# cbrl/BNN-PYNQ

Measured on AMD Instinct MI355X. Metric: images/sec (whole node) CNV-W1A1 CIFAR-10-shape batch, higher is better.
Workload: dtype u1; 1 GPU; cnvW1A1, 131072 synthetic 32x32x3 uint8 images per GPU per step, inputs resident in HBM, params cifar10/cnvW1A1; parallelism=dp1 (batch shards, no data-path collective)

## Files before the change

bnn-pynq_amd/csrc/kernels.hip:

```cpp
#include <hip/hip_runtime.h>
#include <hip/hip_ext.h>
#include <stdint.h>

#include <cstdlib>
#include <cstring>
#include <type_traits>

#define BNN_HD __host__ __device__
#include "act_faults.h"
#include "input_faults.h"
#include "kernels.h"
#include "mem_faults.h"
#include "mem_org.h"
#include "packed_params.h"
static_assert(bnn::kL0TileOffset == (int)bnn::kL0MfmaTileOffset && bnn::kL0BigBytes == (int)bnn::kL0MfmaBigBytes,
              "k_conv0_tile's operand offsets must be the ones packed_params.cpp writes the layer-0 table by");

namespace bnn {
namespace {

typedef const uint32_t __attribute__((address_space(4))) *kptr32;
typedef const uint64_t __attribute__((address_space(4))) *kptr64;

constexpr int kBlock = 256;
// ... 465 lines not shown
      for (int kx = 0; kx < 3; kx++) {
        v8i b[4];
#pragma unroll
        for (int y = 0; y < 4; y++) {
          const uint4 v = P[(2 * r + y) * 30 + cc + kx];
          b[y] = v8i{(int)v.x, (int)v.y, (int)v.z, (int)v.w, 0, 0, 0, 0};
        }
#pragma unroll
        for (int ky = 0; ky < 3; ky++)
#pragma unroll
          for (int mt = 0; mt < 2; mt++)
#pragma unroll
            for (int pt = 0; pt < 2; pt++)
              acc[mt][pt] = __builtin_amdgcn_mfma_scale_f32_32x32x64_f8f6f4(wreg[ky * 3 + kx][mt], b[ky + pt], acc[mt][pt], 4, 4, 0,
                                                                              0x7F7F7F7F, 0, 0x7F7F7F7F);
      }
      uint32_t word[2];
#pragma unroll
      for (int mt = 0; mt < 2; mt++) {
        int v[16];
#pragma unroll
        for (int k = 0; k < 16; k++) v[k] = __float_as_int(fmaxf(acc[mt][0][k], acc[mt][1][k]));
        const uint32_t nf = or_halves(sign_nibbles(v, h));
        const uint32_t pooled = nf & (uint32_t)__builtin_amdgcn_mov_dpp((int)nf, 0xB1, 0xF, 0xF, true);
        word[mt] = ~pooled;
      }
      if (h == 0 && c < 28 && !(c & 1))
        *reinterpret_cast<uint2 *>(out + ((size_t)(img0 + i) * 196 + r * 14 + (c >> 1)) * 2) = make_uint2(word[0], word[1]);
    }
  }
}

constexpr int conv_mfma_row_stride(int win) {
  int ws = win;
  while ((2 * ws - (win - 2)) % 16) ws++;
  return ws;
}
constexpr int conv_mfma_img_stride(int win, int cd) {
  const int ws = conv_mfma_row_stride(win);
  int s = cd * win * ws;
  while ((s - 2 * ((win - 2) / 2 - 1) * ws - (win - 2)) % 16) s++;
  return s;
}

template <int WIN, int CD, int NT, bool POOL, int G>
__global__ __launch_bounds__(256, 2) void k_conv_mfma(const uint32_t *__restrict__ in, uint32_t *__restrict__ out,
                                                       const uint8_t *__restrict__ tab, int n_images) {
  constexpr int WOUT = WIN - 2, RP = WOUT / 2, IPI = RP * WOUT, KH = CD / 2, KS = 9 * KH, NS = 3 * KH, STREAMS = 4 / NT;
  constexpr int PIX = WIN * WIN, DWI = PIX * CD, NPF = (G * DWI + 255) / 256;
  constexpr int WS = conv_mfma_row_stride(WIN), PIXS = WIN * WS, IMGS = conv_mfma_img_stride(WIN, CD);
  static_assert(WOUT % 2 == 0 && IPI % 2 == 0 && (NT == 2 || NT == 4), "tile geometry");
  __shared__ uint4 plane[G * IMGS];
  __shared__ uint32_t lut[256];
  const int tid = threadIdx.x, lane = tid & 63, wave = __builtin_amdgcn_readfirstlane(tid >> 6), mt = wave % NT, c = lane & 31, h = lane >> 5;
  lut[tid] = fp4_pm1((uint32_t)tid);
  const uint4 *__restrict__ wt = reinterpret_cast<const uint4 *>(tab);
  v8i wreg[KS];
#pragma unroll
  for (int ks = 0; ks < KS; ks++) {
    const uint4 v = wt[(ks * NT + mt) * 64 + lane];
    wreg[ks] = v8i{(int)v.x, (int)v.y, (int)v.z, (int)v.w, 0, 0, 0, 0};
  }
  const v16f seed = reinterpret_cast<const v16f *>(tab + (size_t)KS * NT * 64 * 16)[mt * 2 + h];
  const int ngroups = (n_images + G - 1) / G;
  uint32_t pre[NPF];
  auto fetch = [&](int grp) {
    const int img0 = grp * G, lim = min(G, n_images - img0) * DWI;
#pragma unroll
    for (int j = 0; j < NPF; j++) {
      const int d = tid + 256 * j;
      pre[j] = d < lim ? in[(size_t)img0 * DWI + d] : 0u;
    }
  };
  auto slot = [&](int d) {
    const int i = d / DWI, e = d - i * DWI, pix = e / CD, q = e % CD;
    return i * IMGS + q * PIXS + (WS == WIN ? pix : pix / WIN * WS + pix % WIN);
  };
  constexpr int STEP = 32 * STREAMS, DR = STEP / WOUT, DX = STEP % WOUT, PS_LAST = (G - 1) * IMGS + 2 * (RP - 1) * WS + WOUT - 1;
  constexpr bool RAGGED = (G * IPI) % 32 != 0;
  static_assert(DX % 2 == 0 && DR + 1 <= RP, "a lane's column keeps its parity; one row-pair wrap and one image wrap per step");
  const int item0 = (wave / NT) * 32 + c, i0 = item0 / IPI, rem0 = item0 - i0 * IPI, rp0 = rem0 / WOUT, x0 = rem0 - rp0 * WOUT;
  const int ps0 = i0 * IMGS + 2 * rp0 * WS + x0;
  const uint32_t ob0 = (uint32_t)((i0 * (WOUT * WOUT) + (2 * rp0 + h) * WOUT + x0) * NT + mt) * 4;
  if (blockIdx.x < ngroups) fetch(blockIdx.x);
  for (int grp = blockIdx.x; grp < ngroups; grp += gridDim.x) {
    const int img0 = grp * G, nimg = min(G, n_images - img0), nitems = nimg * IPI;
    uint32_t *__restrict__ gout = out + (size_t)img0 * (POOL ? RP * RP : WOUT * WOUT) * NT;
    __syncthreads();
#pragma unroll
    for (int j = 0; j < NPF; j++) {
      const int d = tid + 256 * j;
      if (d < nimg * DWI) {
        const uint32_t bits = pre[j];
        plane[slot(d)] = make_uint4(lut[bits & 255], lut[(bits >> 8) & 255], lut[(bits >> 16) & 255], lut[bits >> 24]);
      }
    }
    if (grp + (int)gridDim.x < ngroups) fetch(grp + gridDim.x);
    __syncthreads();
    int x = x0, rp = rp0, ps = ps0;
    [[maybe_unused]] uint32_t ob = ob0;
    for (int t0 = (wave / NT) * 32; t0 < nitems; t0 += STEP) {
      v16f acc[2] = {seed, seed};
      const uint4 *__restrict__ P = &plane[(RAGGED ? min(ps, PS_LAST) : ps) + h * PIXS];
      auto read = [&](v8i &b, int s, int y) {
        const uint4 v = P[(s / 3) * 2 * PIXS + y * WS + s % 3];
        b = v8i{(int)v.x, (int)v.y, (int)v.z, (int)v.w, 0, 0, 0, 0};
      };
      auto mfma = [&](const v8i (&b)[4], int s, int k) {
        acc[k & 1] = __builtin_amdgcn_mfma_scale_f32_32x32x64_f8f6f4(wreg[((k >> 1) * 3 + s % 3) * KH + s / 3], b[(k >> 1) + (k & 1)], acc[k & 1], 4,
                                                                    4, 0, 0x7F7F7F7F, 0, 0x7F7F7F7F);
      };
      v8i b[2][4];
#pragma unroll
      for (int y = 0; y < 4; y++) read(b[0][y], 0, y);
#pragma unroll
      for (int s = 0; s < NS; s++)
#pragma unroll
        for (int k = 0; k < 6; k++) {
          __builtin_amdgcn_sched_barrier(0);
          mfma(b[s & 1], s, k);
          if (s + 1 < NS && k < 4) read(b[(s + 1) & 1][k], s + 1, k);
        }
      __builtin_amdgcn_sched_barrier(0);
      const bool valid = t0 + c < nitems;
      if constexpr (POOL) {
        int v[16];
#pragma unroll
        for (int k = 0; k < 16; k++) v[k] = __float_as_int(acc[0][k]) & __float_as_int(acc[1][k]);
        const uint32_t nf = or_halves(sign_nibbles(v, h));
        const uint32_t pooled = nf & (uint32_t)__builtin_amdgcn_mov_dpp((int)nf, 0xB1, 0xF, 0xF, true);
        if (valid && h == 0 && !(c & 1)) gout[(size_t)(t0 >> 1) * NT + (c >> 1) * NT + mt] = ~pooled;
      } else {
        uint32_t nf[2];
#pragma unroll
        for (int dy = 0; dy < 2; dy++) {
          int v[16];
#pragma unroll
          for (int k = 0; k < 16; k++) v[k] = __float_as_int(acc[dy][k]);
          nf[dy] = sign_nibbles(v, h);
        }
        const auto sw = __builtin_amdgcn_permlane32_swap(nf[0], nf[1], false, false);
        if (valid) *reinterpret_cast<uint32_t *>(reinterpret_cast<char *>(gout) + ob) = ~(sw[0] | sw[1]);
      }
      x += DX, rp += DR, ps += 2 * DR * WS + DX;
      if constexpr (!POOL) ob += (2 * DR * WOUT + DX) * NT * 4;
      if (x >= WOUT) {
        x -= WOUT, rp += 1, ps += 2 * WS - WOUT;
        if constexpr (!POOL) ob += WOUT * NT * 4;
      }
      if (rp >= RP) rp -= RP, ps += IMGS - 2 * RP * WS;
    }
  }
}

__global__ __launch_bounds__(256) void k_conv_mfma_table(const uint32_t *__restrict__ rows, int row_dw, int ksteps, int tiles,
                                                          int mw, uint8_t *__restrict__ dst) {
  const int idx = blockIdx.x * 256 + threadIdx.x, nw = ksteps * tiles * 64;
  if (idx < nw) {
    const int ks = idx / (tiles * 64), mt = (idx / 64) % tiles, lane = idx & 63, n = 32 * mt + (lane & 31), h = lane >> 5;
    const uint32_t bits = rows[(size_t)n * row_dw + 2 + 2 * ks + h];
    reinterpret_cast<uint4 *>(dst)[idx] = make_uint4(fp4_pm1(bits & 255), fp4_pm1((bits >> 8) & 255), fp4_pm1((bits >> 16) & 255),
                                                     fp4_pm1(bits >> 24));
  } else if (idx < nw + tiles * 32) {
    const int j = idx - nw, mt = j >> 5, h = (j >> 4) & 1, reg = j & 15;
    const int n = 32 * mt + (reg & 3) + 8 * (reg >> 2) + 4 * h;
    long long t = (int)rows[(size_t)n * row_dw];
    t = t < -1 ? -1 : (t > mw + 2 ? mw + 2 : t);
    reinterpret_cast<float *>(dst + (size_t)nw * 16)[j] = (float)(-(mw - 2 * t) - 1);
  }
}

__device__ __forceinline__ uint32_t nibble_spread(uint32_t byte) {
  uint32_t t = byte & 0xFFu;
  t = (t | (t << 12)) & 0x000F000Fu;
  t = (t | (t << 6)) & 0x03030303u;
  return (t | (t << 3)) & 0x11111111u;
}
__device__ __forceinline__ uint4 fp4_planes(const uint32_t *lutz, const uint32_t *luts, uint32_t sg, uint32_t nz) {
  const uint32_t m = sg & nz;
  return make_uint4(lutz[nz & 255] | luts[m & 255], lutz[(nz >> 8) & 255] | luts[(m >> 8) & 255],
                    lutz[(nz >> 16) & 255] | luts[(m >> 16) & 255], lutz[nz >> 24] | luts[m >> 24]);
}
__device__ __forceinline__ void not_fired(const v16f &acc, const v16f &dt, int h, uint32_t &n0, uint32_t &n1) {
  int v[16], u[16];
#pragma unroll
  for (int k = 0; k < 16; k++) {
    v[k] = __float_as_int(acc[k]);
    u[k] = __float_as_int(acc[k] - dt[k]);
  }
  n0 = or_halves(sign_nibbles(v, h));
  n1 = or_halves(sign_nibbles(u, h));
}

template <int WIN, int CD, int NT, bool POOL, int G>
__global__ __launch_bounds__(256, 2) void k_conv_mfma_a2(const uint4 *__restrict__ in, uint32_t *__restrict__ out,
                                                          const uint8_t *__restrict__ tab, int n_images) {
  constexpr int WOUT = WIN - 2, RP = WOUT / 2, IPI = RP * WOUT, KH = CD / 2, KS = 9 * KH, STREAMS = 4 / NT;
  constexpr int PIX = WIN * WIN, QWI = PIX * KH, NPF = (G * QWI + 255) / 256;
  static_assert(WOUT % 2 == 0 && IPI % 2 == 0 && (NT == 2 || NT == 4), "tile geometry");
  __shared__ uint4 plane[G][CD][PIX];
  __shared__ uint32_t lutz[256], luts[256];
  const int tid = threadIdx.x, lane = tid & 63, wave = tid >> 6, mt = wave % NT, c = lane & 31, h = lane >> 5;
  lutz[tid] = nibble_spread((uint32_t)tid) << 1;
  luts[tid] = nibble_spread((uint32_t)tid) << 3;
  const uint4 *__restrict__ wt = reinterpret_cast<const uint4 *>(tab);
  v8i wreg[KS];
#pragma unroll
  for (int ks = 0; ks < KS; ks++) {
    const uint4 v = wt[(ks * NT + mt) * 64 + lane];
    wreg[ks] = v8i{(int)v.x, (int)v.y, (int)v.z, (int)v.w, 0, 0, 0, 0};
  }
  const v16f *__restrict__ cst = reinterpret_cast<const v16f *>(tab + (size_t)KS * NT * 64 * 16);
  const v16f seed = cst[mt * 2 + h], dt = cst[NT * 2 + mt * 2 + h];
  const int ngroups = (n_images + G - 1) / G;
  uint4 pre[NPF];
  auto fetch = [&](int grp) {
    const int img0 = grp * G, lim = min(G, n_images - img0) * QWI;
#pragma unroll
    for (int j = 0; j < NPF; j++) {
      const int d = tid + 256 * j;
      pre[j] = d < lim ? in[(size_t)img0 * QWI + d] : make_uint4(0u, 0u, 0u, 0u);
    }
  };
  if (blockIdx.x < ngroups) fetch(blockIdx.x);
  for (int grp = blockIdx.x; grp < ngroups; grp += gridDim.x) {
    const int img0 = grp * G, nimg = min(G, n_images - img0), nitems = nimg * IPI;
    __syncthreads();
#pragma unroll
    for (int j = 0; j < NPF; j++) {
      const int d = tid + 256 * j;
      if (d < nimg * QWI) {
        const int i = d / QWI, e = d - i * QWI, pix = e / KH, cw = e % KH;
        const uint4 v = pre[j];
        plane[i][2 * cw][pix] = fp4_planes(lutz, luts, v.x, v.z);
        plane[i][2 * cw + 1][pix] = fp4_planes(lutz, luts, v.y, v.w);
      }
    }
    if (grp + (int)gridDim.x < ngroups) fetch(grp + gridDim.x);
    __syncthreads();
    for (int t0 = (wave / NT) * 32; t0 < nitems; t0 += 32 * STREAMS) {
      const int item = min(t0 + c, nitems - 1);
      const int i = item / IPI, rem = item - i * IPI, rp = rem / WOUT, x = rem - rp * WOUT;
      v16f acc[2] = {seed, seed};
#pragma unroll
      for (int kh = 0; kh < KH; kh++) {
        const uint4 *__restrict__ P = &plane[i][kh * 2 + h][2 * rp * WIN + x];
#pragma unroll
        for (int kx = 0; kx < 3; kx++) {
          v8i b[4];
#pragma unroll
          for (int y = 0; y < 4; y++) {
            const uint4 v = P[y * WIN + kx];
            b[y] = v8i{(int)v.x, (int)v.y, (int)v.z, (int)v.w, 0, 0, 0, 0};
          }
#pragma unroll
          for (int ky = 0; ky < 3; ky++)
#pragma unroll
            for (int dy = 0; dy < 2; dy++)
              acc[dy] = __builtin_amdgcn_mfma_scale_f32_32x32x64_f8f6f4(wreg[(ky * 3 + kx) * KH + kh], b[ky + dy], acc[dy], 4, 4, 0,
                                                                         0x7F7F7F7F, 0, 0x7F7F7F7F);
        }
      }
      const bool valid = t0 + c < nitems;
      const size_t img = (size_t)(img0 + i);
      if constexpr (POOL) {
        v16f top;
#pragma unroll
        for (int k = 0; k < 16; k++) top[k] = fmaxf(acc[0][k], acc[1][k]);
        uint32_t n0, n1;
        not_fired(top, dt, h, n0, n1);
        n0 &= (uint32_t)__builtin_amdgcn_mov_dpp((int)n0, 0xB1, 0xF, 0xF, true);
        n1 &= (uint32_t)__builtin_amdgcn_mov_dpp((int)n1, 0xB1, 0xF, 0xF, true);
        const size_t w64 = (img * (RP * RP) + rp * RP + (x >> 1)) * (NT / 2) + mt / 2;
        if (valid && !(x & 1)) out[(w64 * 2 + h) * 2 + (mt & 1)] = h ? ~(n0 ^ n1) : (n0 & n1);
      } else {
        uint32_t n0[2], n1[2];
#pragma unroll
        for (int dy = 0; dy < 2; dy++) not_fired(acc[dy], dt, h, n0[dy], n1[dy]);
        const uint32_t m0 = h ? n0[1] : n0[0], m1 = h ? n1[1] : n1[0];
        const size_t w64 = (img * (WOUT * WOUT) + (2 * rp + h) * WOUT + x) * (NT / 2) + mt / 2;
        if (valid) {
          out[(w64 * 2 + 0) * 2 + (mt & 1)] = m0 & m1;
          out[(w64 * 2 + 1) * 2 + (mt & 1)] = ~(m0 ^ m1);
        }
      }
    }
  }
}

template <bool TT>
__global__ __launch_bounds__(256) void k_conv_mfma_a2_table(const uint32_t *__restrict__ rows, int ksteps, int tiles,
                                                             uint8_t *__restrict__ dst) {
  const int idx = blockIdx.x * 256 + threadIdx.x, nw = ksteps * tiles * 64, row_dw = TT ? 4 + 6 * ksteps : 2 + 2 * ksteps;
  if (idx < nw) {
    const int ks = idx / (tiles * 64), mt = (idx / 64) % tiles, lane = idx & 63, n = 32 * mt + (lane & 31), h = lane >> 5;
    const uint32_t *__restrict__ row = rows + (size_t)n * row_dw;
    uint32_t b1, b2 = 0, b3;
    if constexpr (TT) {
      const uint32_t sg = row[2 + 4 * ks + h], two = row[2 + 4 * ksteps + 2 * ks + h], nz = row[2 + 4 * ks + 2 + h] | two;
      b1 = nz & ~two;
      b2 = two;
      b3 = (sg & nz) | two;
    } else {
      b1 = 0xFFFFFFFFu;
      b3 = row[2 + 2 * ks + h];
    }
// ... 1784 lines not shown
      uint64_t *const w = reinterpret_cast<uint64_t *>(row + 2) + k;
      const uint64_t now = *w ^ mlo;
      if (mlo) *w = now;
      d = __popcll(now ^ was[k]);
    } else {
      uint64_t *const wq = reinterpret_cast<uint64_t *>(row + 2);
      const uint64_t neg = wq[2 * k], nz = wq[2 * k + 1], two = wq[2 * L.kw + k];
      const uint64_t hi = neg ^ mhi, lo = (nz & ~two) ^ mlo, two2 = hi & ~lo;
      if (mlo | mhi) {
        wq[2 * k] = hi;
        wq[2 * k + 1] = hi | lo;
        wq[2 * L.kw + k] = two2;
        if (two2) atomicOr(row + 2 + 6 * L.kw, 1u);
      }
      d = __popcll(hi ^ was[2 * k]) + __popcll(lo ^ (was[2 * k + 1] & ~was[2 * L.kw + k]));
    }
    c = __popcll(mlo) + __popcll(mhi);
  }
#pragma unroll
  for (int s = 32; s >= 1; s >>= 1) {
    c += __shfl_xor(c, s, 64);
    d += __shfl_xor(d, s, 64);
  }
  if ((threadIdx.x & 63) == 0 && (c | d)) {
    unsigned long long *const at = counts + (size_t)run * run_stride + (size_t)L.layer * 4;
    if (c) atomicAdd(at, (unsigned long long)c);
    if (d) atomicAdd(at + 1, (unsigned long long)d);
  }
}

__global__ __launch_bounds__(kBlock) void k_xmem_noise_t(uint8_t *__restrict__ copies, unsigned long long stride, MemNoiseLayer L, unsigned nthr,
                                                         Arith arith, bool signed_bb, const uint16_t *__restrict__ raw, unsigned modules,
                                                         unsigned interleave, unsigned burst, const unsigned long long *__restrict__ seeds,
                                                         unsigned rate, unsigned epoch, unsigned long long *__restrict__ state,
                                                         unsigned long long *__restrict__ counts, unsigned long long run_stride) {
  const unsigned run = blockIdx.y, t = blockIdx.x * kBlock + threadIdx.x;
  uint32_t m = 0;
  unsigned phys = 0;
  if (t < L.rows * nthr) {
    const unsigned n = t / nthr, i = t - n * nthr, mem = n % L.pe, ind = n / L.pe;
    const unsigned long long seed = seeds[run];
    const uint32_t k0 = (uint32_t)seed, k1 = (uint32_t)(seed >> 32), tag = exposure_tag(epoch);
    const unsigned per = (16 + burst - 1) / burst;
    uint32_t hits[3] = {0, 0, 0}, u[3][4], have[3] = {~0u, ~0u, ~0u};
    for (int k = 0; k < 16; k++) {
      int p_ind, p_bit;
      interleave_site((int)interleave, 16, (int)L.tmem, (int)ind, k, &p_ind, &p_bit);
      const uint32_t e = ((mem * L.tmem + (unsigned)p_ind) * nthr + i) * per + (unsigned)p_bit / burst;
#pragma unroll
      for (unsigned md = 0; md < 3; md++) {
        if (md >= modules) break;
        if ((e >> 2) != have[md]) {
          have[md] = e >> 2;
          act_noise_block(k0, k1, L.layer, hardened_draw_word(1, (int)md, (int)burst), have[md], u[md], tag);
        }
        const uint32_t ue = (e & 2) ? ((e & 1) ? u[md][3] : u[md][2]) : ((e & 1) ? u[md][1] : u[md][0]);
        hits[md] |= (ue < rate ? 1u : 0u) << k;
      }
    }
    phys = __popc(hits[0]) + __popc(hits[1]) + __popc(hits[2]);
    unsigned long long *const st = state + (size_t)run * L.rows * nthr + t;
    const unsigned long long before = *st;
    const uint32_t b0 = (uint32_t)before & 0xFFFFu, b1 = (uint32_t)(before >> 16) & 0xFFFFu, b2 = (uint32_t)(before >> 32) & 0xFFFFu;
    const uint32_t a0 = b0 ^ hits[0], a1 = b1 ^ hits[1], a2 = b2 ^ hits[2];
    if (phys) *st = (unsigned long long)a0 | (unsigned long long)a1 << 16 | (unsigned long long)a2 << 32;
    const uint32_t m_before = modules == 3 ? ((b0 & b1) | (b0 & b2) | (b1 & b2)) : b0;
    m = modules == 3 ? ((a0 & a1) | (a0 & a2) | (a1 & a2)) : a0;
    if (m != m_before) {
      uint32_t *const row = reinterpret_cast<uint32_t *>(copies + (size_t)run * stride + L.offset) + (size_t)n * L.row_dwords;
      const int32_t T = (int16_t)(uint16_t)(raw[t] ^ m);
      const uint32_t v = (uint32_t)packed_threshold(arith, signed_bb, 64 * (int)L.kw, T);
      row[i] = v;
      if (nthr == 1) row[1] = v;
    }
  }
  unsigned c = __popc(m);
#pragma unroll
  for (int d = 32; d >= 1; d >>= 1) {
    c += __shfl_xor(c, d, 64);
    phys += __shfl_xor(phys, d, 64);
  }
  if ((threadIdx.x & 63) == 0 && (phys | c)) {
    unsigned long long *const at = counts + (size_t)run * run_stride + (size_t)L.layer * 4 + 2;
    if (phys) atomicAdd(at, (unsigned long long)phys);
    if (c) atomicAdd(at + 1, (unsigned long long)c);
  }
}

inline long long lfc_fused_max() {
  static const long long v = [] {
    const char *e = std::getenv("BNN_MI355X_LFC_FUSED_MAX");
    return e ? std::atoll(e) : 1024LL;
  }();
  return v;
}
inline long long lfc_block_max() {
  static const long long v = [] {
    const char *e = std::getenv("BNN_MI355X_LFC_BLOCK_MAX");
    return e ? std::atoll(e) : 131072LL;
  }();
  return v;
}

inline long long l0_tile_min() {
  static const long long v = [] {
    const char *e = std::getenv("BNN_MI355X_L0_TILE_MIN");
    return e ? std::atoll(e) : 8192LL;
  }();
  return v;
}

constexpr long long kConvMfmaMinW1A2 = 384, kConvMfmaMinW2A2 = 256;
inline long long conv_mfma_min() {
  static const long long v = [] {
    const char *e = std::getenv("BNN_MI355X_CONV_MFMA_MIN");
    return e ? std::atoll(e) : 512LL;
  }();
  return v;
}
template <int ARITH>
inline long long conv_mfma_a2_min() {
  static const long long v = [] {
    const char *e = std::getenv("BNN_MI355X_CONV_MFMA_MIN");
    return e ? std::atoll(e) : (ARITH == AR_TT ? kConvMfmaMinW2A2 : kConvMfmaMinW1A2);
  }();
  return v;
}
template <int ARITH, bool OUT2>
inline const uint8_t *conv_mfma_for(const CnvLaunch &a) {
  if constexpr (ARITH == AR_XNOR && !OUT2) return a.n >= conv_mfma_min() ? a.conv_mfma : nullptr;
  else return a.n >= conv_mfma_a2_min<ARITH>() ? a.conv_mfma : nullptr;
}
constexpr long long kTailMfmaMinW1A1 = 3072, kTailMfmaMinW1A2 = 3072, kTailMfmaMinW2A2 = 1024;
constexpr int kTailMfmaStages = 0xF0;
template <int ARITH>
inline long long tail_mfma_min() {
  static const long long v = [] {
    const char *e = std::getenv("BNN_MI355X_TAIL_MFMA_MIN");
    return e ? std::atoll(e) : (ARITH == AR_XNOR ? kTailMfmaMinW1A1 : ARITH == AR_TB ? kTailMfmaMinW1A2 : kTailMfmaMinW2A2);
  }();
  return v;
}
template <int ARITH>
inline const uint8_t *tail_mfma_for(const CnvLaunch &a) {
  if (a.done_flag && a.n == 1) return nullptr;
  return a.n >= tail_mfma_min<ARITH>() ? a.conv_mfma : nullptr;
}
inline unsigned persistent_grid(long long units, long long cap) {
  const long long per = (units + cap - 1) / cap;
  return (unsigned)((units + per - 1) / per);
}
constexpr long long kConvMfmaGrid = 512;
constexpr int kConvMfmaImgsL1 = 2, kConvMfmaImgs = 8;
constexpr int kTailMfmaImgsL4 = 32, kTailMfmaImgsL5 = 32, kTailMfmaImgsFc = 128;
constexpr long long kTailMfmaGrid8 = 256;
#define BNN_TAIL_MFMA(A2, KS, NT, CONV, WAVES, G, cap, in, out, tab)                                                               \
  hipLaunchKernelGGL((k_tail_mfma<A2, KS, NT, CONV, WAVES, G>), dim3(persistent_grid((n + (G) - 1) / (G), (cap))), dim3(64 * (WAVES)), 0, s, \
                     in, out, tab, (int)n)

inline int gpb_for(long long items, int groups) { return (items + kBlock - 1) / kBlock >= 2048 ? groups : 1; }

inline bool narrow_for(long long items, int groups32, long long limit) { return ((items + kBlock - 1) / kBlock) * groups32 < limit; }
constexpr long long kNarrowLimitCnv = 8192, kNarrowLimitLfc = 512;
constexpr long long kFcLastWaveMax = 32768;
constexpr long long kPixelLaneMax = 512;
constexpr long long kCnvTailMax = 1024;

inline dim3 grid_for(long long items, int groups) {
  const long long item_blocks = (items + kBlock - 1) / kBlock;
  return dim3((unsigned)(((item_blocks + 7) / 8) * 8 * groups));
}

#define BNN_LAUNCH(kern, grid, stream, ...)                                   \
  do {                                                                        \
    if ((grid).x > 0) hipLaunchKernelGGL(kern, grid, dim3(kBlock), 0, stream, __VA_ARGS__); \
  } while (0)
#define BNN_STAGE(kern32, kern8, items, groups32, in, out, rows)                                                                   \
  do {                                                                                                                             \
    const long long it_ = (items);                                                                                                 \
    if (narrow_for(it_, (groups32), narrow_limit)) BNN_LAUNCH(kern8, grid_for(it_, (groups32) * 4), s, in, out, rows, (int)it_, (groups32) * 4, 1); \
    else BNN_LAUNCH(kern32, grid_for(it_, (groups32) / gpb_for(it_, (groups32))), s, in, out, rows, (int)it_, (groups32), gpb_for(it_, (groups32))); \
  } while (0)
#define BNN_MARK(ev, i, stream)                          \
  do {                                                   \
    if (ev) (void)hipEventRecord((ev)[i], stream);       \
  } while (0)

template <int ARITH, bool OUT2, bool TWO = false>
void run_cnv_t(const CnvLaunch &a) {
  const long long n = a.n, narrow_limit = kNarrowLimitCnv;
  uint32_t *A = reinterpret_cast<uint32_t *>(a.buf0), *B = reinterpret_cast<uint32_t *>(a.buf1);
  const uint64_t *A64 = reinterpret_cast<const uint64_t *>(a.buf0), *B64 = reinterpret_cast<const uint64_t *>(a.buf1);
  hipStream_t s = a.stream;
  BNN_MARK(a.events, 0, s);
  if (a.l0_mfma) {
    const dim3 g0((unsigned)((n * 900 + kBlock - 1) / kBlock));
    if (a.last_stage >= 0) {
      if (n >= l0_tile_min()) BNN_LAUNCH((k_conv0_tile<OUT2>), dim3((unsigned)((n + kL0Imgs - 1) / kL0Imgs)), s, a.images, A, a.l0_mfma, (int)n);
      else BNN_LAUNCH((k_conv0_mfma<OUT2>), g0, s, a.images, A, a.l0_mfma, (int)(n * 900));
    }
  } else {
    if (a.last_stage >= 0) BNN_LAUNCH((k_conv0<OUT2>), grid_for(n * 900, 2 / gpb_for(n * 900, 2)), s, a.images, A, a.rows[0], (int)(n * 900), 2, gpb_for(n * 900, 2));
  }
  BNN_MARK(a.events, 1, s);
  if constexpr (ARITH == AR_XNOR && !OUT2) {
    const bool pix = n <= kPixelLaneMax;
    const uint8_t *const cm = conv_mfma_for<ARITH, OUT2>(a);
    const dim3 g1(persistent_grid((n + kConvMfmaImgsL1 - 1) / kConvMfmaImgsL1, kConvMfmaGrid)),
        gm(persistent_grid((n + kConvMfmaImgs - 1) / kConvMfmaImgs, kConvMfmaGrid));
    if (a.last_stage >= 1) {
      if (a.l1_literal) {
        BNN_LAUNCH(k_l1_literal, dim3((unsigned)((n * 784 + kBlock - 1) / kBlock)), s, A64, reinterpret_cast<uint64_t *>(B), a.rows[1], (int)(n * 784));
      } else if (a.l1_mfma) {
        const long long pairs = (n + 1) / 2;
        hipLaunchKernelGGL(k_l1_mfma, dim3((unsigned)(pairs < 512 ? pairs : 512)), dim3(256), 0, s, reinterpret_cast<const uint32_t *>(a.buf0), B,
                           a.l1_mfma, (int)n);
      } else if (cm) {
        hipLaunchKernelGGL((k_conv_mfma<30, 2, 2, true, kConvMfmaImgsL1>), g1, dim3(256), 0, s, reinterpret_cast<const uint32_t *>(a.buf0), B, cm,
                           (int)n);
      } else if (pix) BNN_LAUNCH((k_vec_x<9, true, 1, 30, 8, true>), grid_for(n * 784, 8), s, A64, B, a.rows[1], (int)(n * 784), 8, 1);
      else BNN_STAGE((k_quad_x<1, 30, true>), (k_quad_x<1, 30, true, 8>), n * 196, 2, A64, B, a.rows[1]);
    }
    BNN_MARK(a.events, 2, s);
    if (a.last_stage >= 2) {
      if (cm) hipLaunchKernelGGL((k_conv_mfma<14, 2, 4, false, kConvMfmaImgs>), gm, dim3(256), 0, s, B, A, cm + kConvMfmaL2Off, (int)n);
      else if (pix) BNN_LAUNCH((k_vec_x<9, true, 1, 14, 8>), grid_for(n * 144, 16), s, B64, A, a.rows[2], (int)(n * 144), 16, 1);
      else BNN_STAGE((k_quad_x<1, 14, false>), (k_quad_x<1, 14, false, 8>), n * 36, 4, B64, A, a.rows[2]);
    }
    BNN_MARK(a.events, 3, s);
    if (a.last_stage >= 3) {
      if (cm) hipLaunchKernelGGL((k_conv_mfma<12, 4, 4, true, kConvMfmaImgs>), gm, dim3(256), 0, s, A, B, cm + kConvMfmaL3Off, (int)n);
      else if (pix) BNN_LAUNCH((k_vec_x<18, true, 2, 12, 8, true>), grid_for(n * 100, 16), s, A64, B, a.rows[3], (int)(n * 100), 16, 1);
      else BNN_STAGE((k_quad_x<2, 12, true>), (k_quad_x<2, 12, true, 8>), n * 25, 4, A64, B, a.rows[3]);
    }
    BNN_MARK(a.events, 4, s);
    const uint8_t *const tm = tail_mfma_for<ARITH>(a);
    const uint32_t *const A32 = A, *const B32 = B;
    if (!tm && n <= kCnvTailMax && !a.events && a.last_stage >= kCnvStages - 1) {
      hipLaunchKernelGGL(k_cnv_tail, dim3((unsigned)n), dim3(512), 0, s, B64, a.scores, a.classes, a.rows[4], a.rows[5], a.rows[6],
                         a.rows[7], a.rows[8], a.number_class, n == 1 ? a.done_flag : nullptr, a.done_seq);
      return;
    }
    if (a.last_stage >= 4) {
      if (tm && (kTailMfmaStages & 16)) BNN_TAIL_MFMA(false, 18, 8, true, 8, kTailMfmaImgsL4, kTailMfmaGrid8, B32, A, tm + kTailMfmaL4Off);
      else BNN_STAGE((k_vec_x<18, true, 2, 5>), (k_vec_x<18, true, 2, 5, 8>), n * 9, 8, B64, A, a.rows[4]);
    }
    BNN_MARK(a.events, 5, s);
    if (a.last_stage >= 5) {
      if (tm && (kTailMfmaStages & 32)) BNN_TAIL_MFMA(false, 36, 8, false, 8, kTailMfmaImgsL5, kTailMfmaGrid8, A32, B, tm + kTailMfmaL5Off);
      else BNN_STAGE((k_vec_x<36, false, 1, 1>), (k_vec_x<36, false, 1, 1, 8>), n, 8, A64, B, a.rows[5]);
    }
    BNN_MARK(a.events, 6, s);
    if (a.last_stage >= 6) {
      if (tm && (kTailMfmaStages & 64)) BNN_TAIL_MFMA(false, 4, 16, false, 4, kTailMfmaImgsFc, kConvMfmaGrid, B32, A, tm + kTailMfmaL6Off);
      else BNN_STAGE((k_vec_x<4, false, 1, 1>), (k_vec_x<4, false, 1, 1, 8>), n, 16, B64, A, a.rows[6]);
    }
    BNN_MARK(a.events, 7, s);
    if (a.last_stage >= 7) {
      if (tm && (kTailMfmaStages & 128)) BNN_TAIL_MFMA(false, 8, 16, false, 8, kTailMfmaImgsFc, kTailMfmaGrid8, A32, B, tm + kTailMfmaL7Off);
      else BNN_STAGE((k_vec_x<8, false, 1, 1>), (k_vec_x<8, false, 1, 1, 8>), n, 16, A64, B, a.rows[7]);
    }
    BNN_MARK(a.events, 8, s);
  } else {
    const bool pix = n <= kPixelLaneMax;
    const uint8_t *const cm = conv_mfma_for<ARITH, OUT2>(a);
    const uint4 *const A128 = reinterpret_cast<const uint4 *>(a.buf0), *const B128 = reinterpret_cast<const uint4 *>(a.buf1);
    const dim3 g1(persistent_grid((n + kConvMfmaImgsL1 - 1) / kConvMfmaImgsL1, kConvMfmaGrid)),
        gm(persistent_grid((n + kConvMfmaImgs - 1) / kConvMfmaImgs, kConvMfmaGrid));
    if (a.last_stage >= 1) {
      if (cm) hipLaunchKernelGGL((k_conv_mfma_a2<30, 2, 2, true, kConvMfmaImgsL1>), g1, dim3(256), 0, s, A128, B, cm, (int)n);
      else if (pix) BNN_LAUNCH((k_vec<ARITH, 9, OUT2, true, 1, 30, 8, true, TWO>), grid_for(n * 784, 8), s, A64, B, a.rows[1], (int)(n * 784), 8, 1);
      else BNN_STAGE((k_quad<ARITH, 1, 30, true, OUT2, 32, TWO>), (k_quad<ARITH, 1, 30, true, OUT2, 8, TWO>), n * 196, 2, A64, B, a.rows[1]);
    }
    BNN_MARK(a.events, 2, s);
    if (a.last_stage >= 2) {
      if (cm) hipLaunchKernelGGL((k_conv_mfma_a2<14, 2, 4, false, kConvMfmaImgs>), gm, dim3(256), 0, s, B128, A, cm + kConvMfmaA2L2Off, (int)n);
      else if (pix) BNN_LAUNCH((k_vec<ARITH, 9, OUT2, true, 1, 14, 8, false, TWO>), grid_for(n * 144, 16), s, B64, A, a.rows[2], (int)(n * 144), 16, 1);
      else BNN_STAGE((k_quad<ARITH, 1, 14, false, OUT2, 32, TWO>), (k_quad<ARITH, 1, 14, false, OUT2, 8, TWO>), n * 36, 4, B64, A, a.rows[2]);
    }
    BNN_MARK(a.events, 3, s);
    if (a.last_stage >= 3) {
      if (cm) hipLaunchKernelGGL((k_conv_mfma_a2<12, 4, 4, true, kConvMfmaImgs>), gm, dim3(256), 0, s, A128, B, cm + kConvMfmaA2L3Off, (int)n);
      else if (pix) BNN_LAUNCH((k_vec<ARITH, 18, OUT2, true, 2, 12, 8, true, TWO>), grid_for(n * 100, 16), s, A64, B, a.rows[3], (int)(n * 100), 16, 1);
      else BNN_STAGE((k_quad<ARITH, 2, 12, true, OUT2, 32, TWO>), (k_quad<ARITH, 2, 12, true, OUT2, 8, TWO>), n * 25, 4, A64, B, a.rows[3]);
    }
    BNN_MARK(a.events, 4, s);
    const uint8_t *const tm = tail_mfma_for<ARITH>(a);
    if constexpr (!TWO) {
      if (!tm && n <= kCnvTailMax && !a.events && a.last_stage >= kCnvStages - 1) {
        hipLaunchKernelGGL((k_cnv_tail_a2<ARITH>), dim3((unsigned)n), dim3(512), 0, s, B64, a.scores, a.classes, a.rows[4], a.rows[5],
                           a.rows[6], a.rows[7], a.rows[8], a.number_class, n == 1 ? a.done_flag : nullptr, a.done_seq);
        return;
      }
    }
    if (a.last_stage >= 4) {
      if (tm && (kTailMfmaStages & 16)) BNN_TAIL_MFMA(true, 18, 8, true, 8, kTailMfmaImgsL4, kTailMfmaGrid8, B128, A, tm + kTailMfmaA2L4Off);
      else BNN_STAGE((k_vec<ARITH, 18, OUT2, true, 2, 5, 32, false, TWO>), (k_vec<ARITH, 18, OUT2, true, 2, 5, 8, false, TWO>), n * 9, 8, B64, A, a.rows[4]);
    }
    BNN_MARK(a.events, 5, s);
    if (a.last_stage >= 5) {
      if (tm && (kTailMfmaStages & 32)) BNN_TAIL_MFMA(true, 36, 8, false, 8, kTailMfmaImgsL5, kTailMfmaGrid8, A128, B, tm + kTailMfmaA2L5Off);
      else BNN_STAGE((k_vec<ARITH, 36, OUT2, false, 1, 1, 32, false, TWO>), (k_vec<ARITH, 36, OUT2, false, 1, 1, 8, false, TWO>), n, 8, A64, B, a.rows[5]);
    }
    BNN_MARK(a.events, 6, s);
    if (a.last_stage >= 6) {
      if (tm && (kTailMfmaStages & 64)) BNN_TAIL_MFMA(true, 4, 16, false, 4, kTailMfmaImgsFc, kConvMfmaGrid, B128, A, tm + kTailMfmaA2L6Off);
      else BNN_STAGE((k_vec<ARITH, 4, OUT2, false, 1, 1, 32, false, TWO>), (k_vec<ARITH, 4, OUT2, false, 1, 1, 8, false, TWO>), n, 16, B64, A, a.rows[6]);
    }
    BNN_MARK(a.events, 7, s);
    if (a.last_stage >= 7) {
      if (tm && (kTailMfmaStages & 128)) BNN_TAIL_MFMA(true, 8, 16, false, 8, kTailMfmaImgsFc, kTailMfmaGrid8, A128, B, tm + kTailMfmaA2L7Off);
      else BNN_STAGE((k_vec<ARITH, 8, OUT2, false, 1, 1, 32, false, TWO>), (k_vec<ARITH, 8, OUT2, false, 1, 1, 8, false, TWO>), n, 16, A64, B, a.rows[7]);
    }
    BNN_MARK(a.events, 8, s);
  }
  if (a.last_stage >= 8) {
    if (n <= kFcLastWaveMax) BNN_LAUNCH((k_fclast_wave<ARITH, 8, TWO>), dim3((unsigned)((n + 3) / 4)), s, B64, a.scores, a.classes, a.rows[8], (int)n, a.number_class);
    else BNN_LAUNCH((k_fclast<ARITH, 8, TWO>), grid_for(n, 1), s, B64, a.scores, a.classes, a.rows[8], (int)n, a.number_class);
  }
  BNN_MARK(a.events, 9, s);
}

template <int ARITH, bool OUT2>
int matrix_stages_t(const CnvLaunch &a) {
  const bool cm = conv_mfma_for<ARITH, OUT2>(a) != nullptr;
  bool l1 = cm;
  if constexpr (ARITH == AR_XNOR && !OUT2) l1 = !a.l1_literal && (a.l1_mfma || cm);
  return (a.l0_mfma ? 1 : 0) | (l1 ? 2 : 0) | (cm ? 12 : 0) | (tail_mfma_for<ARITH>(a) ? kTailMfmaStages : 0);
}

#define BNN_MULTI(kern, ipi, groups32, in, out, rows, RES)                                                               \
  do {                                                                                                                   \
    const long long it_ = (long long)a.total * (ipi);                                                                    \
    const int gpb_ = gpb_for(it_, (groups32));                                                                           \
    const MultiArgs ma_{a.segs, (unsigned)(a.stride / 4), (ipi), (RES) ? a.n : 0};                                       \
    dim3 g_ = grid_for((long long)a.max_len * (ipi), (groups32) / gpb_);                                                 \
    g_.y = (unsigned)a.nsegs;                                                                                            \
    BNN_LAUNCH(kern, g_, s, in, out, rows, (int)it_, (groups32), gpb_, ma_);                                             \
  } while (0)

template <int ARITH, bool OUT2, bool TWO = false>
void run_cnv_multi_t(const MultiLaunch &a) {
  uint32_t *A = reinterpret_cast<uint32_t *>(a.buf0), *B = reinterpret_cast<uint32_t *>(a.buf1);
  const uint64_t *A64 = reinterpret_cast<const uint64_t *>(a.buf0), *B64 = reinterpret_cast<const uint64_t *>(a.buf1);
  hipStream_t s = a.stream;
  const auto in = [&](int l) { return a.first <= l && l <= a.last; };
  if (in(0) && a.l0_mfma) {
    const MultiArgs ma{a.segs, (unsigned)(a.stride / 4), 1, 0};
    BNN_LAUNCH((k_conv0_tile<OUT2, true>), dim3((unsigned)((a.max_len + kL0Imgs - 1) / kL0Imgs), (unsigned)a.nsegs), s, a.images, A,
               a.l0_mfma, 0, ma);
  } else if (in(0)) {
    BNN_MULTI((k_conv0<OUT2, true>), 900, 2, a.images, A, a.rows[0], false);
  }
  if constexpr (ARITH == AR_XNOR && !OUT2) {
    if (in(1)) BNN_MULTI((k_quad_x<1, 30, true, 32, true>), 196, 2, A64, B, a.rows[1], false);
    if (in(2)) BNN_MULTI((k_quad_x<1, 14, false, 32, true>), 36, 4, B64, A, a.rows[2], false);
    if (in(3)) BNN_MULTI((k_quad_x<2, 12, true, 32, true>), 25, 4, A64, B, a.rows[3], false);
    if (in(4)) BNN_MULTI((k_vec_x<18, true, 2, 5, 32, false, true>), 9, 8, B64, A, a.rows[4], false);
    if (in(5)) BNN_MULTI((k_vec_x<36, false, 1, 1, 32, false, true>), 1, 8, A64, B, a.rows[5], false);
    if (in(6)) BNN_MULTI((k_vec_x<4, false, 1, 1, 32, false, true>), 1, 16, B64, A, a.rows[6], false);
    if (in(7)) BNN_MULTI((k_vec_x<8, false, 1, 1, 32, false, true>), 1, 16, A64, B, a.rows[7], false);
  } else {
    if (in(1)) BNN_MULTI((k_quad<ARITH, 1, 30, true, OUT2, 32, TWO, true>), 196, 2, A64, B, a.rows[1], false);
    if (in(2)) BNN_MULTI((k_quad<ARITH, 1, 14, false, OUT2, 32, TWO, true>), 36, 4, B64, A, a.rows[2], false);
    if (in(3)) BNN_MULTI((k_quad<ARITH, 2, 12, true, OUT2, 32, TWO, true>), 25, 4, A64, B, a.rows[3], false);
    if (in(4)) BNN_MULTI((k_vec<ARITH, 18, OUT2, true, 2, 5, 32, false, TWO, true>), 9, 8, B64, A, a.rows[4], false);
    if (in(5)) BNN_MULTI((k_vec<ARITH, 36, OUT2, false, 1, 1, 32, false, TWO, true>), 1, 8, A64, B, a.rows[5], false);
    if (in(6)) BNN_MULTI((k_vec<ARITH, 4, OUT2, false, 1, 1, 32, false, TWO, true>), 1, 16, B64, A, a.rows[6], false);
    if (in(7)) BNN_MULTI((k_vec<ARITH, 8, OUT2, false, 1, 1, 32, false, TWO, true>), 1, 16, A64, B, a.rows[7], false);
  }
  if (!in(8)) return;
  const MultiArgs ma{a.segs, (unsigned)(a.stride / 4), 1, a.n};
  dim3 g = grid_for(a.max_len, 1);
  g.y = (unsigned)a.nsegs;
  BNN_LAUNCH((k_fclast<ARITH, 8, TWO, true>), g, s, B64, nullptr, a.classes, a.rows[8], a.total, a.number_class, ma);
}

#define BNN_WIN(kern, ipi, groups32, out, rows)                                                                          \
  do {                                                                                                                   \
    const long long it_ = (long long)a.total * (ipi);                                                                    \
    const int gpb_ = gpb_for(it_, (groups32));                                                                           \
    const MultiArgs ma_{a.segs, (unsigned)(a.stride / 4), (ipi), 0};                                                     \
    dim3 g_ = grid_for((long long)a.max_len * (ipi), (groups32) / gpb_);                                                 \
    g_.y = (unsigned)a.nsegs;                                                                                            \
// ... 439 lines not shown
```

Measured before the change: 40.84 million images/s.

## Add ping-pong two-team MFMA conv kernel overlapping plane expansion with tile compute

```diff
diff --git a/bnn-pynq_amd/csrc/kernels.hip b/bnn-pynq_amd/csrc/kernels.hip
--- a/bnn-pynq_amd/csrc/kernels.hip
+++ b/bnn-pynq_amd/csrc/kernels.hip
@@ -641,6 +641,167 @@
     }
   }
 }
+
+#ifndef BNN_CONV_PP_X1
+#define BNN_CONV_PP_X1 2
+#endif
+#ifndef BNN_CONV_PP_X2
+#define BNN_CONV_PP_X2 2
+#endif
+#ifndef BNN_CONV_PP_X3
+#define BNN_CONV_PP_X3 2
+#endif
+constexpr int conv_pp_x(int win) { return win == 30 ? BNN_CONV_PP_X1 : win == 14 ? BNN_CONV_PP_X2 : BNN_CONV_PP_X3; }
+#define BNN_PP_BARRIER()                   \
+  do {                                     \
+    __builtin_amdgcn_sched_barrier(0);     \
+    __builtin_amdgcn_s_barrier();          \
+    __builtin_amdgcn_sched_barrier(0);     \
+  } while (0)
+
+template <int WIN, int CD, int NT, bool POOL, int G>
+__global__ __launch_bounds__(512) void k_conv_mfma_pp(const uint32_t *__restrict__ in, uint32_t *__restrict__ out,
+                                                       const uint8_t *__restrict__ tab, int n_images) {
+  constexpr int WOUT = WIN - 2, RP = WOUT / 2, IPI = RP * WOUT, KH = CD / 2, KS = 9 * KH, NS = 3 * KH, STREAMS = 4 / NT;
+  constexpr int PIX = WIN * WIN, DWI = PIX * CD, NPF = (G * DWI + 255) / 256;
+  constexpr int WS = conv_mfma_row_stride(WIN), PIXS = WIN * WS, IMGS = conv_mfma_img_stride(WIN, CD);
+  static_assert(WOUT % 2 == 0 && IPI % 2 == 0 && (NT == 2 || NT == 4), "tile geometry");
+  constexpr int T = ((G * IPI + 31) / 32 + STREAMS - 1) / STREAMS, X = conv_pp_x(WIN), PH = X + 2 * T, D = (PH / 2) | 1;
+  constexpr int BARRIERS_TEAM0 = PH + D, BARRIERS_TEAM1 = D + PH;
+  static_assert(X % 2 == 0 && X >= 2 && X <= NPF, "an even number of expansion phases");
+  static_assert(D % 2 == 1 && D >= X && D + X <= PH, "team 1 lags by an odd number of phases; its expansion falls into team 0's tile loop");
+  static_assert(BARRIERS_TEAM0 == BARRIERS_TEAM1, "both teams execute the same number of barriers");
+  __shared__ struct {
+    uint4 plane[2][G * IMGS];
+    uint32_t lut[256];
+  } lds;
+  const int tid = threadIdx.x, lane = tid & 63, wave = __builtin_amdgcn_readfirstlane(tid >> 6), team = wave >> 2, tw = wave & 3;
+  const int ttid = tid & 255, mt = tw % NT, c = lane & 31, h = lane >> 5;
+  if (tid < 256) lds.lut[tid] = fp4_pm1((uint32_t)tid);
+  uint4 *const plane = lds.plane[team];
+  const uint32_t *const lut = lds.lut;
+  const uint4 *__restrict__ wt = reinterpret_cast<const uint4 *>(tab);
+  v8i wreg[KS];
+#pragma unroll
+  for (int ks = 0; ks < KS; ks++) {
+    const uint4 v = wt[(ks * NT + mt) * 64 + lane];
+    wreg[ks] = v8i{(int)v.x, (int)v.y, (int)v.z, (int)v.w, 0, 0, 0, 0};
+  }
+  const v16f seed = reinterpret_cast<const v16f *>(tab + (size_t)KS * NT * 64 * 16)[mt * 2 + h];
+  const int ngroups = (n_images + G - 1) / G, npairs = (ngroups + 1) / 2;
+  uint32_t pre[NPF];
+  auto fetch = [&](int grp) {
+    const int img0 = grp * G, lim = min(G, n_images - img0) * DWI;
+#pragma unroll
+    for (int j = 0; j < NPF; j++) {
+      const int d = ttid + 256 * j;
+      pre[j] = d < lim ? in[(size_t)img0 * DWI + d] : 0u;
+    }
+  };
+  auto slot = [&](int d) {
+    const int i = d / DWI, e = d - i * DWI, pix = e / CD, q = e % CD;
+    return i * IMGS + q * PIXS + (WS == WIN ? pix : pix / WIN * WS + pix % WIN);
+  };
+  constexpr int STEP = 32 * STREAMS, DR = STEP / WOUT, DX = STEP % WOUT, PS_LAST = (G - 1) * IMGS + 2 * (RP - 1) * WS + WOUT - 1;
+  constexpr bool RAGGED = (G * IPI) % 32 != 0 || T * STREAMS * 32 != G * IPI;
+  static_assert(DX % 2 == 0 && DR + 1 <= RP, "a lane's column keeps its parity; one row-pair wrap and one image wrap per step");
+  const int item0 = (tw / NT) * 32 + c, i0 = item0 / IPI, rem0 = item0 - i0 * IPI, rp0 = rem0 / WOUT, x0 = rem0 - rp0 * WOUT;
+  const int ps0 = i0 * IMGS + 2 * rp0 * WS + x0;
+  const uint32_t ob0 = (uint32_t)((i0 * (WOUT * WOUT) + (2 * rp0 + h) * WOUT + x0) * NT + mt) * 4;
+  __builtin_amdgcn_s_waitcnt(0x0F70);
+  fetch(2 * blockIdx.x + team);
+  __syncthreads();
+  if (team == 1) {
+#pragma unroll 1
+    for (int i = 0; i < D; i++) BNN_PP_BARRIER();
+  }
+#pragma unroll 1
+  for (int pair = blockIdx.x; pair < npairs; pair += gridDim.x) {
+    const int grp = 2 * pair + team, img0 = grp * G, nimg = max(0, min(G, n_images - img0)), nitems = nimg * IPI;
+    uint32_t *__restrict__ gout = out + (size_t)img0 * (POOL ? RP * RP : WOUT * WOUT) * NT;
+#pragma unroll
+    for (int e = 0; e < X; e++) {
+#pragma unroll
+      for (int j = e * NPF / X; j < (e + 1) * NPF / X; j++) {
+        const int d = ttid + 256 * j;
+        if (d < nimg * DWI) {
+          const uint32_t bits = pre[j];
+          plane[slot(d)] = make_uint4(lut[bits & 255], lut[(bits >> 8) & 255], lut[(bits >> 16) & 255], lut[bits >> 24]);
+        }
+      }
+      if (e == X - 1 && pair + (int)gridDim.x < npairs) fetch(2 * (pair + (int)gridDim.x) + team);
+      asm volatile("s_waitcnt lgkmcnt(0)" ::: "memory");
+      BNN_PP_BARRIER();
+    }
+    int x = x0, rp = rp0, ps = ps0;
+    [[maybe_unused]] uint32_t ob = ob0;
+    const uint4 *__restrict__ Pt = &plane[(RAGGED ? min(ps, PS_LAST) : ps) + h * PIXS];
+    auto read = [&](v8i &b, int s, int y) {
+      const uint4 v = Pt[(s / 3) * 2 * PIXS + y * WS + s % 3];
+      b = v8i{(int)v.x, (int)v.y, (int)v.z, (int)v.w, 0, 0, 0, 0};
+    };
+    v8i b[2][4];
+#pragma unroll
+    for (int y = 0; y < 4; y++) read(b[0][y], 0, y);
+#pragma unroll 1
+    for (int it = 0; it < T; it++) {
+      const int t0 = (tw / NT) * 32 + it * STEP;
+      v16f acc[2] = {seed, seed};
+      auto mfma = [&](const v8i (&bb)[4], int s, int k) {
+        acc[k & 1] = __builtin_amdgcn_mfma_scale_f32_32x32x64_f8f6f4(wreg[((k >> 1) * 3 + s % 3) * KH + s / 3], bb[(k >> 1) + (k & 1)], acc[k & 1], 4,
+                                                                    4, 0, 0x7F7F7F7F, 0, 0x7F7F7F7F);
+      };
+#pragma unroll
+      for (int s = 0; s < NS; s++)
+#pragma unroll
+        for (int k = 0; k < 6; k++) {
+          __builtin_amdgcn_sched_barrier(0);
+          mfma(b[s & 1], s, k);
+          if (s + 1 < NS && k < 4) read(b[(s + 1) & 1][k], s + 1, k);
+        }
+      asm volatile("" ::"v"(acc[0]), "v"(acc[1]));
+      BNN_PP_BARRIER();
+      const bool valid = t0 + c < nitems;
+      if constexpr (POOL) {
+        int v[16];
+#pragma unroll
+        for (int k = 0; k < 16; k++) v[k] = __float_as_int(acc[0][k]) & __float_as_int(acc[1][k]);
+        const uint32_t nf = or_halves(sign_nibbles(v, h));
+        const uint32_t pooled = nf & (uint32_t)__builtin_amdgcn_mov_dpp((int)nf, 0xB1, 0xF, 0xF, true);
+        if (valid && h == 0 && !(c & 1)) gout[(size_t)(t0 >> 1) * NT + (c >> 1) * NT + mt] = ~pooled;
+      } else {
+        uint32_t nf[2];
+#pragma unroll
+        for (int dy = 0; dy < 2; dy++) {
+          int v[16];
+#pragma unroll
+          for (int k = 0; k < 16; k++) v[k] = __float_as_int(acc[dy][k]);
+          nf[dy] = sign_nibbles(v, h);
+        }
+        const auto sw = __builtin_amdgcn_permlane32_swap(nf[0], nf[1], false, false);
+        if (valid) *reinterpret_cast<uint32_t *>(reinterpret_cast<char *>(gout) + ob) = ~(sw[0] | sw[1]);
+      }
+      x += DX, rp += DR, ps += 2 * DR * WS + DX;
+      if constexpr (!POOL) ob += (2 * DR * WOUT + DX) * NT * 4;
+      if (x >= WOUT) {
+        x -= WOUT, rp += 1, ps += 2 * WS - WOUT;
+        if constexpr (!POOL) ob += WOUT * NT * 4;
+      }
+      if (rp >= RP) rp -= RP, ps += IMGS - 2 * RP * WS;
+      if (it + 1 < T) {
+        Pt = &plane[(RAGGED ? min(ps, PS_LAST) : ps) + h * PIXS];
+#pragma unroll
+        for (int y = 0; y < 4; y++) read(b[0][y], 0, y);
+      }
+      BNN_PP_BARRIER();
+    }
+  }
+  if (team == 0) {
+#pragma unroll 1
+    for (int i = 0; i < D; i++) BNN_PP_BARRIER();
+  }
+}
+#undef BNN_PP_BARRIER
 
 __global__ __launch_bounds__(256) void k_conv_mfma_table(const uint32_t *__restrict__ rows, int row_dw, int ksteps, int tiles,
                                                           int mw, uint8_t *__restrict__ dst) {
@@ -2731,6 +2892,23 @@
 }
 constexpr long long kConvMfmaGrid = 512;
 constexpr int kConvMfmaImgsL1 = 2, kConvMfmaImgs = 8;
+constexpr long long kConvPpMin = 200000;
+constexpr bool kConvPpL1 = true, kConvPpL2 = true, kConvPpL3 = true;
+inline long long conv_pp_min() {
+  static const long long v = [] {
+    const char *e = std::getenv("BNN_MI355X_CONV_PP_MIN");
+    return e ? std::atoll(e) : kConvPpMin;
+  }();
+  return v;
+}
+inline long long conv_pp_grid() {
+  static const long long v = [] {
+    const char *e = std::getenv("BNN_MI355X_CONV_PP_GRID");
+    const long long g = e ? std::atoll(e) : 256LL;
+    return g < 1 ? 1LL : g > 256 ? 256LL : g;
+  }();
+  return v;
+}
 constexpr int kTailMfmaImgsL4 = 32, kTailMfmaImgsL5 = 32, kTailMfmaImgsFc = 128;
 constexpr long long kTailMfmaGrid8 = 256;
 #define BNN_TAIL_MFMA(A2, KS, NT, CONV, WAVES, G, cap, in, out, tab)                                                               \
@@ -2787,6 +2965,9 @@
     const uint8_t *const cm = conv_mfma_for<ARITH, OUT2>(a);
     const dim3 g1(persistent_grid((n + kConvMfmaImgsL1 - 1) / kConvMfmaImgsL1, kConvMfmaGrid)),
         gm(persistent_grid((n + kConvMfmaImgs - 1) / kConvMfmaImgs, kConvMfmaGrid));
+    const bool pp = cm && n >= conv_pp_min();
+    const dim3 p1(persistent_grid(((n + kConvMfmaImgsL1 - 1) / kConvMfmaImgsL1 + 1) / 2, conv_pp_grid())),
+        pm(persistent_grid(((n + kConvMfmaImgs - 1) / kConvMfmaImgs + 1) / 2, conv_pp_grid()));
     if (a.last_stage >= 1) {
       if (a.l1_literal) {
         BNN_LAUNCH(k_l1_literal, dim3((unsigned)((n * 784 + kBlock - 1) / kBlock)), s, A64, reinterpret_cast<uint64_t *>(B), a.rows[1], (int)(n * 784));
@@ -2794,6 +2975,9 @@
         const long long pairs = (n + 1) / 2;
         hipLaunchKernelGGL(k_l1_mfma, dim3((unsigned)(pairs < 512 ? pairs : 512)), dim3(256), 0, s, reinterpret_cast<const uint32_t *>(a.buf0), B,
                            a.l1_mfma, (int)n);
+      } else if (pp && kConvPpL1) {
+        hipLaunchKernelGGL((k_conv_mfma_pp<30, 2, 2, true, kConvMfmaImgsL1>), p1, dim3(512), 0, s, reinterpret_cast<const uint32_t *>(a.buf0), B, cm,
+                           (int)n);
       } else if (cm) {
         hipLaunchKernelGGL((k_conv_mfma<30, 2, 2, true, kConvMfmaImgsL1>), g1, dim3(256), 0, s, reinterpret_cast<const uint32_t *>(a.buf0), B, cm,
                            (int)n);
@@ -2802,13 +2986,15 @@
     }
     BNN_MARK(a.events, 2, s);
     if (a.last_stage >= 2) {
-      if (cm) hipLaunchKernelGGL((k_conv_mfma<14, 2, 4, false, kConvMfmaImgs>), gm, dim3(256), 0, s, B, A, cm + kConvMfmaL2Off, (int)n);
+      if (pp && kConvPpL2) hipLaunchKernelGGL((k_conv_mfma_pp<14, 2, 4, false, kConvMfmaImgs>), pm, dim3(512), 0, s, B, A, cm + kConvMfmaL2Off, (int)n);
+      else if (cm) hipLaunchKernelGGL((k_conv_mfma<14, 2, 4, false, kConvMfmaImgs>), gm, dim3(256), 0, s, B, A, cm + kConvMfmaL2Off, (int)n);
       else if (pix) BNN_LAUNCH((k_vec_x<9, true, 1, 14, 8>), grid_for(n * 144, 16), s, B64, A, a.rows[2], (int)(n * 144), 16, 1);
       else BNN_STAGE((k_quad_x<1, 14, false>), (k_quad_x<1, 14, false, 8>), n * 36, 4, B64, A, a.rows[2]);
     }
     BNN_MARK(a.events, 3, s);
     if (a.last_stage >= 3) {
-      if (cm) hipLaunchKernelGGL((k_conv_mfma<12, 4, 4, true, kConvMfmaImgs>), gm, dim3(256), 0, s, A, B, cm + kConvMfmaL3Off, (int)n);
+      if (pp && kConvPpL3) hipLaunchKernelGGL((k_conv_mfma_pp<12, 4, 4, true, kConvMfmaImgs>), pm, dim3(512), 0, s, A, B, cm + kConvMfmaL3Off, (int)n);
+      else if (cm) hipLaunchKernelGGL((k_conv_mfma<12, 4, 4, true, kConvMfmaImgs>), gm, dim3(256), 0, s, A, B, cm + kConvMfmaL3Off, (int)n);
       else if (pix) BNN_LAUNCH((k_vec_x<18, true, 2, 12, 8, true>), grid_for(n * 100, 16), s, A64, B, a.rows[3], (int)(n * 100), 16, 1);
       else BNN_STAGE((k_quad_x<2, 12, true>), (k_quad_x<2, 12, true, 8>), n * 25, 4, A64, B, a.rows[3]);
     }
```

Result: no change. 41.36 million images/s, median of 3 (+1.3%).
